# robertknight/rten

Measured on NVIDIA H100. Metric: resnet50_fp32_inferences_per_sec, higher is better.
Workload: dtype f32(tf32 mma, explicit opt-in)

## Files before the change

rten_b200/csrc/umma_gemm.cu:

```cuda
#include <cuda.h>
#include <cuda_runtime.h>

#include <algorithm>
#include <array>
#include <cmath>
#include <vector>
#include <cmath>
#include <cstdint>
#include <cstdio>
#include <cstdlib>

#include "math.cuh"
#include "ptx.cuh"
#include "rowops.h"
#include "umma_gemm.h"
#include "umma_kernel.cuh"

namespace rtb {

typedef CUresult (*EncodeTiledFn)(CUtensorMap*, CUtensorMapDataType, cuuint32_t, void*, const cuuint64_t*,
                                  const cuuint64_t*, const cuuint32_t*, const cuuint32_t*, CUtensorMapInterleave,
                                  CUtensorMapSwizzle, CUtensorMapL2promotion, CUtensorMapFloatOOBfill);

static EncodeTiledFn get_encode(rten_ctx* ctx) {
// ... 18 lines not shown
        }
    }
    for (int i = 0; i < rank; i++)
        if (od.dims[i] < 1 || od.dims[i] > 0xFFFFFFFFll) return false;
    return true;
}

bool encode_map(rten_ctx* ctx, CUtensorMap* map, const OperandDesc& od, int esize, bool is_f32,
                const uint32_t box[4], const uint32_t estr[4]) {
    EncodeTiledFn enc = get_encode(ctx);
    if (!enc) return false;
    cuuint64_t dims[4];
    cuuint64_t strides[3];
    cuuint32_t b[4], es[4];
    for (int i = 0; i < 4; i++) {
        dims[i] = (cuuint64_t)od.dims[i];
        b[i] = box[i];
        es[i] = estr[i];
    }
    for (int i = 1; i < 4; i++) {
        long long s = od.strides[i] * esize;
        if (s == 0 || od.dims[i] == 1) s = 16;
        strides[i - 1] = (cuuint64_t)s;
    }
    CUresult r = enc(map, is_f32 ? CU_TENSOR_MAP_DATA_TYPE_FLOAT32 : CU_TENSOR_MAP_DATA_TYPE_UINT8, 4,
                     const_cast<void*>(od.base), dims, strides, b, es, CU_TENSOR_MAP_INTERLEAVE_NONE,
                     CU_TENSOR_MAP_SWIZZLE_128B, CU_TENSOR_MAP_L2_PROMOTION_L2_256B,
                     CU_TENSOR_MAP_FLOAT_OOB_FILL_NONE);
    return r == CUDA_SUCCESS;
}

static void pick_conv_tile(const ConvGeom& g, int& tw, int& th, int& tb) {
    double best = -1.0;
    tw = th = tb = 1;
    for (int w = 1; w <= std::min(g.OW, 128); w++) {
        if (w * g.sx > 256) break;
        for (int h = 1; h <= std::min(g.OH, 128 / w); h++) {
            if (h * g.sy > 256) break;
            int b = std::min(g.B, 128 / (w * h));
            if (b < 1) continue;
            long long tiles = (long long)((g.OW + w - 1) / w) * ((g.OH + h - 1) / h) * ((g.B + b - 1) / b);
            double eff = (double)g.B * g.OH * g.OW / ((double)tiles * 128.0);
            if (eff > best + 1e-9 || (eff > best - 1e-9 && w > tw)) {
                best = eff;
                tw = w;
                th = h;
                tb = b;
            }
        }
    }
}

struct Plan {
    int bn = 32, splitk = 1, nbuf = 1;
    bool halo = false;
    int T = 0;
};

static Plan halo_plan(int bn, int T) {
    Plan pl;
    pl.halo = true;
    pl.bn = bn;
    pl.T = T;
    return pl;
}

struct Prepared {
    KParams p;
    uint32_t abox[4], aes[4], bbox_k;
    uint32_t pbox[4], pes[4];
    uint32_t a_rows;
    long long batch;
    OperandDesc od, ord;
    uint32_t dbox[4];
    int tma_store, res_tma;
    int wide;
    int chain_bytes;
    int step;
    int esize, kelems;
};

constexpr int SK_CNT_INTS = 1 << 16;
static int smem_budget_for(int n_stg) { return 227 * 1024 - SMEM_FIXED_BYTES - n_stg * STG_BYTES; }
static int wide_stages(int stage_bytes, int chain_bytes) {
    return std::min(MAX_STAGES, (227 * 1024 - WIDE_SMEM_FIXED_BYTES - chain_bytes) / stage_bytes);
}
static bool is_wide(int bn) { return bn > ACC_STRIDE; }

static Epi pick_epilogue(const GemmLaunch& L, int tma_store, int res_tma, int splitk) {
    const EpilogueDesc& e = L.epi;
    auto aligned = [](const void* ptr) { return (reinterpret_cast<uintptr_t>(ptr) & 15) == 0; };
    bool fast = tma_store && (L.N % 32) == 0 && !getenv("RTEN_B200_NO_FAST") && e.bias_kind != 2 &&
                (e.r == nullptr || res_tma) && (e.bias_kind != 1 || aligned(e.bias));
    if (L.kind == 1)
        fast = fast && (!(e.za || e.za8) || aligned(e.colsum)) && (!e.zb || e.zb_len == 1 || (e.zb_len == L.N && aligned(e.zb))) &&
               (!e.scale || e.scale_len == 1 || (e.scale_len == L.N && aligned(e.scale)));
    if (!fast) return Epi::Generic;
    const bool gelu = e.act > 1;
    if (!getenv("RTEN_B200_NO_PLAIN") && e.act <= 7) {
        if (L.kind == 0 && e.alpha == 1.0f && !e.range && (e.r == nullptr || e.r_scale == 1.0f))
            return gelu ? Epi::PlainF32Gelu : Epi::PlainF32;
        if (L.kind == 1 && e.scale && !e.za && !e.zb && (e.scale_len == 1 || e.scale_len == L.N) && splitk == 1 &&
            (!e.za8 || e.colsum))
            return gelu ? Epi::PlainI8Gelu : Epi::PlainI8;
    }
    return gelu ? Epi::FastGelu : Epi::Fast;
}

static const char* epi_name(Epi v) {
    static const char* const names[] = {"Generic", "Fast", "FastGelu", "PlainF32", "PlainF32Gelu", "PlainI8", "PlainI8Gelu"};
    return names[(int)v];
}

static bool is_plain_f32(Epi v) { return v == Epi::PlainF32 || v == Epi::PlainF32Gelu; }

struct PlanShape {
    long long tiles_n, units_m, tiles, units;
    int kb_per, stage_bytes, stages, n_stg;
};

static bool plan_shape(const Prepared& q, const Plan& pl, PlanShape& ps) {
    const KParams& p = q.p;
    if (pl.splitk < 1) return false;
    if (is_wide(pl.bn)) {
        if ((pl.bn != 128 && pl.bn != 256) || !q.wide || pl.splitk != 1) return false;
        if (pl.bn == 256 && q.p.epi.act > 1) return false;
    } else if (pl.bn < 16 || pl.bn % 32 || pl.bn % q.step) {
        return false;
    }
    if (pl.nbuf < (q.res_tma ? 2 : 1) || pl.nbuf > 4) return false;
    ps.tiles_n = q.chain_bytes ? 1 : (p.N + pl.bn - 1) / pl.bn;
    ps.units_m = p.tiles_m;
    ps.tiles = ps.units_m * ps.tiles_n * q.batch;
    ps.units = ps.tiles * pl.splitk;
    if (ps.units > 0x7FFFFFFFll) return false;
    ps.kb_per = (p.k_blocks + pl.splitk - 1) / pl.splitk;
    if (pl.splitk > 1) {
        if (pl.bn % 32 || (long long)(pl.splitk - 1) * ps.kb_per >= p.k_blocks) return false;
        if (ps.tiles * 2 > SK_CNT_INTS) return false;
    }
    ps.n_stg = 2 * pl.nbuf;
    ps.stage_bytes = A_STAGE_BYTES + pl.bn * KBYTES;
    ps.stages = is_wide(pl.bn) ? wide_stages(ps.stage_bytes, q.chain_bytes) : std::min(MAX_STAGES, smem_budget_for(ps.n_stg) / ps.stage_bytes);
    if (ps.stages < 2) return false;
    return true;
}

static double plan_cost(const Prepared& q, const Plan& pl, const PlanShape& ps, int num_sms) {
    const double active = (double)std::min<long long>(ps.units, num_sms);
    const double waves = std::ceil((double)ps.units / num_sms);
    const double bw = std::min(64.0, 7400.0 / active);
    const double mmas = 4.0;
    const double t_kb = std::max(mmas * std::max(42.0, (double)pl.bn), ps.stage_bytes / bw);
    double t_stage = std::max(t_kb, 320.0 + mmas * 42.0);
    t_stage = std::max(t_stage, 2300.0 / ps.stages);
    const double mainloop = ps.kb_per * t_stage;
    const double epi = is_wide(pl.bn) ? (pl.bn / 32.0) * 400.0 + 600.0 : (pl.bn / 32.0) * 350.0 / 2.0 + 600.0;
    double unit = (is_wide(pl.bn) ? mainloop + epi : std::max(mainloop, epi)) + 1500.0;
    double cost = waves * unit + 2500.0;
    if (pl.splitk > 1) cost += epi * (1.0 + 0.25 * pl.splitk) + 1500.0;

    return cost;
}

static void enumerate_plans(const Prepared& q, int num_sms, std::vector<std::pair<double, Plan>>& out) {
    const KParams& p = q.p;
    const int nmax = (p.N + q.step - 1) / q.step * q.step;
    static const int splits[] = {1, 2, 3, 4, 5, 6, 8, 10, 12, 16};
    for (int bn : {32, 64, 128, 256}) {
        if (bn > nmax && bn != 32) break;
        for (int sk : splits) {
            Plan pl;
            pl.bn = bn;
            pl.splitk = sk;
            if (sk > 1 && p.k_blocks / sk < 4) continue;
            const int kb_per = (p.k_blocks + sk - 1) / sk;
            pl.nbuf = (q.res_tma || kb_per < 24) ? 2 : 1;
            PlanShape ps;
            if (is_wide(bn)) {
                pl.nbuf = 2;
            } else if (pl.nbuf == 2) {
                PlanShape ps2;
                const bool ok2 = plan_shape(q, pl, ps2);
                pl.nbuf = 3;
                if (!plan_shape(q, pl, ps) || (ps.stages < 3 && !(ok2 && ps.stages == ps2.stages))) pl.nbuf = 2;
            }
            if (!plan_shape(q, pl, ps)) continue;
            if (sk > 1 && ps.tiles >= 2 * num_sms) continue;
            if (ps.stages < 2) continue;
            out.emplace_back(plan_cost(q, pl, ps, num_sms), pl);
        }
    }
    std::sort(out.begin(), out.end(), [](const std::pair<double, Plan>& x, const std::pair<double, Plan>& y) {
        return x.first < y.first;
    });
}

static rten_status prepare_launch(rten_ctx* ctx, const GemmLaunch& L, Prepared& q) {
    const int esize = L.kind == 0 ? 4 : 1;
    const int kelems = KBYTES / esize;
    if (!tma_compatible(L.a, esize, 4) || !tma_compatible(L.b, esize, 4)) return RTEN_ERR_UNSUPPORTED_VALUE;
    if (L.M <= 0 || L.N <= 0 || L.K <= 0) return RTEN_ERR_UNSUPPORTED_VALUE;
    q.esize = esize;
    q.kelems = kelems;
    KParams& p = q.p;
    memset(&p, 0, sizeof(p));
    p.M = L.M;
    p.N = L.N;
    p.K = L.K;
    p.z0 = L.z0;
    p.z1 = L.z1;
    p.kelems = kelems;
    p.conv = L.conv;
    p.epi = L.epi;
    p.c_blocks = 1;
    p.kw = 1;
    for (int i = 0; i < 4; i++) q.aes[i] = 1;
    if (L.conv) {
        const ConvGeom& g = L.g;
        pick_conv_tile(g, p.tw, p.th, p.tb);
        p.tiles_x = (g.OW + p.tw - 1) / p.tw;
        p.tiles_y = (g.OH + p.th - 1) / p.th;
        int tiles_b = (g.B + p.tb - 1) / p.tb;
        p.tiles_m = p.tiles_x * p.tiles_y * tiles_b;
        p.OH = g.OH;
        p.OW = g.OW;
        p.Bn = g.B;
        p.sy = g.sy;
        p.sx = g.sx;
        p.dy = g.dy;
        p.dx = g.dx;
        p.pt = g.pt;
        p.pl = g.pl;
        p.kw = g.kw;
        p.c_blocks = (g.C + kelems - 1) / kelems;
        p.k_blocks = g.kh * g.kw * p.c_blocks;
        p.z0 = p.z1 = 1;
        q.abox[0] = kelems;
        q.abox[1] = p.tw * g.sx;
        q.abox[2] = p.th * g.sy;
        q.abox[3] = p.tb;
        q.aes[1] = g.sx;
        q.aes[2] = g.sy;
        q.a_rows = p.tw * p.th * p.tb;
        q.batch = 1;
    } else {
        p.tiles_m = (L.M + BM - 1) / BM;
        p.k_blocks = (L.K + kelems - 1) / kelems;
        q.abox[0] = kelems;
        q.abox[1] = BM;
        q.abox[2] = 1;
        q.abox[3] = 1;
        q.a_rows = BM;
        q.batch = (long long)L.z0 * L.z1;
        p.a_bcast0 = (L.a.dims[2] == 1 && L.z0 > 1) ? 1 : 0;
        p.a_bcast1 = (L.a.dims[3] == 1 && L.z1 > 1) ? 1 : 0;
        p.b_bcast0 = (L.b.dims[2] == 1 && L.z0 > 1) ? 1 : 0;
        p.b_bcast1 = (L.b.dims[3] == 1 && L.z1 > 1) ? 1 : 0;
    }
    OperandDesc& od = q.od;
    OperandDesc& ord = q.ord;
    q.dbox[0] = 32;
    q.dbox[1] = q.dbox[2] = q.dbox[3] = 1;
// ... 85 lines not shown
    }
    return RTEN_OK;
}

static rten_status launch_plan(rten_ctx* ctx, const GemmLaunch& L, const Prepared& q, const Plan& pl, bool verbose,
                               void* ws = nullptr) {
    PlanShape ps;
    if (!plan_shape(q, pl, ps)) return RTEN_ERR_UNSUPPORTED_VALUE;
    KParams p = q.p;
    p.bn = pl.bn;
    p.splitk = pl.splitk;
    p.nbuf = pl.nbuf;
    p.tma_store = q.tma_store;
    p.res_tma = q.res_tma ? 1 : 0;
    p.kb_per = ps.kb_per;
    p.tiles_n = (int)ps.tiles_n;
    p.tiles_total = (int)ps.tiles;
    p.units_total = (int)ps.units;
    p.d_tiles_n.set(p.tiles_n);
    p.d_tiles_m.set(p.tiles_m);
    p.d_z0.set(p.z0);
    p.d_tiles_x.set(p.conv ? p.tiles_x : 1);
    p.d_tiles_y.set(p.conv ? p.tiles_y : 1);
    p.d_tiles_total.set(p.tiles_total);
    p.d_c_blocks.set(p.c_blocks);
    p.d_kw.set(p.kw);
    p.d_tw.set(p.conv ? p.tw : 1);
    p.d_th.set(p.conv ? p.th : 1);
    p.stage_bytes = ps.stage_bytes;
    p.tx_bytes = q.a_rows * KBYTES + p.bn * KBYTES;
    p.stages = ps.stages;
    p.sgn = L.kind == 0 ? 0 : (L.a_signed ? 1 : 0) | (L.b_signed ? 2 : 0);
    if (p.splitk > 1) {
        RTB_TRY(ensure_splitk_counters(ctx));
        if (!ws) RTB_TRY(temp_alloc(ctx, splitk_ws_bytes(ps, pl), &ws));
        p.sk_ws = reinterpret_cast<uint32_t*>(ws);
        p.sk_cnt = reinterpret_cast<int*>(ctx->sk_counters);
    }

    uint32_t bbox[4] = {(uint32_t)q.kelems, (uint32_t)p.bn, 1, 1}, bes[4] = {1, 1, 1, 1}, des[4] = {1, 1, 1, 1};
    TmaMaps m;
    if (!encode_map(ctx, &m.a, L.a, q.esize, L.kind == 0, q.abox, q.aes)) return RTEN_ERR_UNSUPPORTED_VALUE;
    if (!encode_map(ctx, &m.b, L.b, q.esize, L.kind == 0, bbox, bes)) return RTEN_ERR_UNSUPPORTED_VALUE;
    m.d = m.r = m.a2 = m.a_proj = m.b_proj = m.a2_proj = m.w2 = m.z = m.a;
    p.x3_cb = L.x3_cb;
    if (L.x3_cb && !encode_map(ctx, &m.a2, L.a_lo, q.esize, true, q.abox, q.aes)) return RTEN_ERR_UNSUPPORTED_VALUE;
    if (p.kb_proj) {
        p.x3_cb_proj = L.proj.x3_cb;
        if (!encode_map(ctx, &m.a_proj, L.proj.a, 4, true, q.pbox, q.pes) ||
            !encode_map(ctx, &m.b_proj, L.proj.b, 4, true, bbox, bes) ||
            (L.proj.x3_cb && !encode_map(ctx, &m.a2_proj, L.proj.a_lo, 4, true, q.pbox, q.pes)))
            return RTEN_ERR_UNSUPPORTED_VALUE;
    }
    if (p.tma_store && !encode_map(ctx, &m.d, q.od, 4, true, q.dbox, des)) {
        p.tma_store = 0;
        p.res_tma = 0;
        m.d = m.a;
    }
    if (p.res_tma && !encode_map(ctx, &m.r, q.ord, 4, true, q.dbox, des)) {
        p.res_tma = 0;
        m.r = m.a;
    }
    const Epi epi = pick_epilogue(L, p.tma_store, p.res_tma, p.splitk);
    if (epi == Epi::Generic && (L.kind == 1 || L.epi.act > 1)) p.res_tma = 0;
    if (q.chain_bytes) {
        const GemmLaunch::Chain& c = L.chain;
        const uint32_t wbox[4] = {32, (uint32_t)c.N2, 1, 1}, zbox[4] = {32, q.dbox[1], q.dbox[2], q.dbox[3]};
        if (epi != Epi::PlainF32 || (L.epi.r && !p.res_tma) || !encode_map(ctx, &m.w2, c.w, 4, true, wbox, des) ||
            !encode_map(ctx, &m.z, c.z, 4, true, zbox, des))
            return RTEN_ERR_UNSUPPORTED_VALUE;
        p.chain_n2 = c.N2;
        p.chain_passes = (L.N + p.bn - 1) / p.bn;
        p.chain_act = c.act;
        p.chain_bias = c.bias;
    }

    if (verbose)
        fprintf(stderr, "[umma_gemm] kind=%d conv=%d M=%d N=%d K=%d kb=%d kb_proj=%d tiles_m=%d bn=%d splitk=%d units=%d stages=%d tma_store=%d res_tma=%d nbuf=%d box=%dx%dx%d epi=%s%s\n",
                L.kind, L.conv, L.M, L.N, L.K, p.k_blocks, p.kb_proj, p.tiles_m, p.bn, p.splitk, p.units_total, p.stages,
                p.tma_store, p.res_tma, p.nbuf, p.tw, p.th, p.tb, epi_name(epi),
                p.chain_n2 == 64 ? " chain=64" : p.chain_n2 == 128 ? " chain=128" : "");
    if ((is_wide(p.bn) || p.kb_proj || L.epi.bias2) && !is_plain_f32(epi)) return RTEN_ERR_UNSUPPORTED_VALUE;
    const size_t smem_bytes = (size_t)p.stages * p.stage_bytes + q.chain_bytes +
                              (is_wide(p.bn) ? WIDE_SMEM_FIXED_BYTES : ps.n_stg * STG_BYTES + SMEM_FIXED_BYTES);
    using Kernel = void (*)(TmaMaps, KParams);
    static const Kernel narrow[2][7] = {
        {umma_gemm_kernel<0, Epi::Generic>, umma_gemm_kernel<0, Epi::Fast>, umma_gemm_kernel<0, Epi::FastGelu>,
         umma_gemm_kernel<0, Epi::PlainF32>, umma_gemm_kernel<0, Epi::PlainF32Gelu>, nullptr, nullptr},
        {umma_gemm_kernel<1, Epi::Generic>, umma_gemm_kernel<1, Epi::Fast>, umma_gemm_kernel<1, Epi::FastGelu>, nullptr,
         nullptr, umma_gemm_kernel<1, Epi::PlainI8>, umma_gemm_kernel<1, Epi::PlainI8Gelu>}};
    const Kernel kern = !is_wide(p.bn)              ? narrow[L.kind][(int)epi]
                        : p.chain_n2 == 64         ? umma_wide_kernel<Epi::PlainF32, 64>
                        : p.chain_n2 == 128        ? umma_wide_kernel<Epi::PlainF32, 128>
                        : epi == Epi::PlainF32Gelu ? umma_wide_kernel<Epi::PlainF32Gelu>
                                                   : umma_wide_kernel<Epi::PlainF32>;

    const int threads = is_wide(p.bn) ? WIDE_THREADS : NUM_THREADS;
    return launch(ctx, "umma_gemm launch", kern, {std::min(p.units_total, ctx->num_sms), threads, smem_bytes, 227 * 1024, true}, m, p);
}

static std::vector<long long> tune_key(const GemmLaunch& L, const Prepared& q) {
    const EpilogueDesc& e = L.epi;
    std::vector<long long> k = {L.kind, L.conv, L.M, L.N, L.K, L.z0, L.z1, q.tma_store, q.res_tma, e.act, e.bias_kind,
                                e.r != nullptr, (e.za != nullptr || e.za8 != nullptr), e.zb != nullptr, e.scale != nullptr,
                                L.a.strides[1], L.b.strides[1], L.x3_cb};
    if (L.conv) {
        const ConvGeom& g = L.g;
        for (long long v : {g.B, g.H, g.W, g.C, g.OH, g.OW, g.kh, g.kw, g.sy, g.sx, g.dy, g.dx, g.pt, g.pl}) k.push_back(v);
    }
    if (L.proj.C > 0) {
        const GemmLaunch::Projection& pr = L.proj;
        for (int64_t v : {(int64_t)-1, (int64_t)pr.C, (int64_t)pr.stride, (int64_t)pr.x3_cb, pr.a.dims[1], pr.a.dims[2],
                          pr.a.strides[1], pr.a.strides[2], pr.a.strides[3], pr.b.strides[1]})
            k.push_back(v);
    }
    return k;
}

static std::array<int, 3> plan_record(const Plan& pl) {
    return pl.halo ? std::array<int, 3>{-1, pl.bn, pl.T} : std::array<int, 3>{pl.bn, pl.splitk, pl.nbuf};
}

static Plan plan_from_record(const std::array<int, 3>& r) {
    if (r[0] < 0) return halo_plan(r[1], r[2]);
    Plan pl;
    pl.bn = r[0];
    pl.splitk = r[1];
    pl.nbuf = r[2];
    return pl;
}

void tune_cache_load(rten_ctx* ctx, const char* path) {
    FILE* f = fopen(path, "r");
    if (!f) return;
    char line[2048];
    while (fgets(line, sizeof(line), f)) {
        std::vector<long long> key;
        std::array<int, 3> plan{};
        char* p = line;
        bool in_plan = false;
        int np = 0;
        while (*p) {
            while (*p == ' ') p++;
            if (*p == '|') {
                in_plan = true;
                p++;
                continue;
            }
            if (*p == '\n' || *p == 0) break;
            char* end = nullptr;
            const long long v = strtoll(p, &end, 10);
            if (end == p) break;
            if (in_plan) {
                if (np < 3) plan[np] = (int)v;
                np++;
            } else {
                key.push_back(v);
            }
            p = end;
        }
        if (np == 3 && !key.empty()) ctx->tune_cache[key] = plan;
    }
    fclose(f);
}

void tune_cache_save(rten_ctx* ctx, const char* path) {
    FILE* f = fopen(path, "w");
// ... 111 lines not shown
    for (size_t i = 0; i < ncand; i++) {
        PlanShape ps;
        if (plan_shape(q, cands[i].second, ps)) ws_max = std::max(ws_max, splitk_ws_bytes(ps, cands[i].second));
    }
    void* ws = nullptr;
    if (ws_max) {
        RTB_TRY(ensure_splitk_counters(ctx));
        RTB_TRY(temp_alloc(ctx, ws_max, &ws));
        cudaStreamSynchronize(ctx->stream);
    }
    cudaEvent_t e0, e1;
    cudaEventCreate(&e0);
    cudaEventCreate(&e1);
    auto time_plan = [&](const Plan& x, int n) -> double {
        if (run_plan(ctx, L, q, x, false, ws) != RTEN_OK) return -1.0;
        cudaEventRecord(e0, ctx->stream);
        bool ok = true;
        for (int r = 0; r < n && ok; r++) ok = run_plan(ctx, L, q, x, false, ws) == RTEN_OK;
        cudaEventRecord(e1, ctx->stream);
        if (cudaEventSynchronize(e1) != cudaSuccess || !ok) return -1.0;
        float t = 0.f;
        cudaEventElapsedTime(&t, e0, e1);
        return (double)t / n;
    };
    double best_ms = 1e30;
    int reps = 4;
    std::vector<std::pair<double, size_t>> timed;
    for (size_t i = 0; i < ncand; i++) {
        const Plan& x = cands[i].second;
        double ms = time_plan(x, reps);
        if (ms < 0) continue;
        timed.emplace_back(ms, i);
        if (verbose)
            fprintf(stderr, "[autotune] bn=%d splitk=%d nbuf=%d model=%.0f -> %.2f us\n", x.bn, x.splitk, x.nbuf,
                    cands[i].first, ms * 1e3);
        if (ms < best_ms) {
            best_ms = ms;
            plan = x;
        }
        reps = std::max(4, std::min(32, (int)(0.15 / std::max(best_ms, 1e-3))));
    }
    std::sort(timed.begin(), timed.end());
    best_ms = 1e30;
    for (size_t k = 0; k < std::min<size_t>(3, timed.size()); k++) {
        const Plan& x = cands[timed[k].second].second;
        const double again = time_plan(x, 2 * reps);
        const double ms = again < 0 ? timed[k].first : again;
        if (ms < best_ms) {
            best_ms = ms;
            plan = x;
        }
    }
    for (const auto& s : HALO_SHAPES) {
        const Plan x = halo_plan(s[0], s[1]);
        if (!halo || x.bn > L.N) continue;
        double ms = time_plan(x, reps);
        if (ms > 0 && ms < best_ms * 1.05) ms = time_plan(x, 2 * reps);
        if (verbose && ms > 0) fprintf(stderr, "[autotune] halo bn=%d T=%d -> %.2f us\n", x.bn, x.T, ms * 1e3);
        if (ms > 0 && ms < best_ms * 0.97) {
            best_ms = ms;
            plan = x;
        }
    }
    cudaEventDestroy(e0);
    cudaEventDestroy(e1);
    ctx->tune_cache[tune_key(L, q)] = plan_record(plan);
    return RTEN_OK;
}

rten_status launch_umma_gemm(rten_ctx* ctx, const GemmLaunch& L) {
    const bool verbose = getenv("RTEN_B200_VERBOSE") != nullptr;
    const char* force_bn = getenv("RTEN_B200_FORCE_BN");
    const char* force_sk = getenv("RTEN_B200_FORCE_SPLITK");
    const char* halo_on = getenv("RTEN_B200_HALO");
    const bool halo = L.conv && L.kind == 0 && L.g.kh * L.g.kw > 1 && !L.x3_cb && !L.proj.C && !getenv("RTEN_B200_NO_HALO");
    Prepared q;
    if (L.chain.N2 > 0) {
        if (L.kind != 0 || ctx->f32_mode != RTEN_F32_TF32 || L.x3_cb || getenv("RTEN_B200_NO_CHAIN"))
            return RTEN_ERR_UNSUPPORTED_VALUE;
        RTB_TRY(prepare_launch(ctx, L, q));
        Plan pl;
        pl.bn = 128;
        pl.nbuf = 2;
        return launch_plan(ctx, L, q, pl, verbose);
    }
    if (L.kind == 0 && ctx->f32_mode == RTEN_F32_TF32X3) return launch_tf32x3(ctx, L);
    int hbn, hT;
    if (halo && halo_on && atoi(halo_on) != 0 && halo_model_shape(ctx, L, hbn, hT)) {
        const rten_status hs = run_plan(ctx, L, q, halo_plan(hbn, hT), verbose);
        if (hs != RTEN_ERR_UNSUPPORTED_VALUE) return hs;
    }
    RTB_TRY(prepare_launch(ctx, L, q));
    const bool forced = force_bn || force_sk;
    if (!forced && !ctx->tune_cache.empty()) {
        auto hit = ctx->tune_cache.find(tune_key(L, q));
        if (hit != ctx->tune_cache.end()) {
            const Plan pl = plan_from_record(hit->second);
            PlanShape ps;
            if (pl.halo ? halo && halo_shape_fits(L, pl.bn, pl.T) : plan_shape(q, pl, ps)) return run_plan(ctx, L, q, pl, verbose);
            if (verbose) fprintf(stderr, "[umma_gemm] recorded plan no longer valid for this problem: re-planning\n");
            ctx->tune_cache.erase(hit);
        }
    }
    std::vector<std::pair<double, Plan>> cands;
    enumerate_plans(q, ctx->num_sms, cands);
    if (cands.empty()) return RTEN_ERR_UNSUPPORTED_VALUE;
    Plan plan = cands[0].second;
    if (forced) {
        bool found = false;
        for (const auto& c : cands) {
            const Plan& x = c.second;
            if (force_bn && x.bn != atoi(force_bn)) continue;
            if (force_sk && x.splitk != atoi(force_sk)) continue;
            plan = x;
            found = true;
            break;
        }
        if (!found) {
            ctx->forced_misses++;
            if (verbose) fprintf(stderr, "[umma_gemm] no valid plan matches the forced fields: using the model's choice\n");
            if (getenv("RTEN_B200_FORCE_STRICT"))
                return fail(ctx, RTEN_ERR_INVALID_VALUE, "no launch plan matches the forced RTEN_B200_FORCE_* fields");
        } else {
            ctx->forced_hits++;
        }
    } else if (ctx->autotune) {
        RTB_TRY(autotune(ctx, L, q, cands, halo, verbose, plan));
    }
    return run_plan(ctx, L, q, plan, verbose);
}

}
```

rten_b200/csrc/umma_kernel.cuh:

```cuda
#pragma once
#include <cuda.h>
#include <cuda_runtime.h>

#include <cstdint>

#include "math.cuh"
#include "ptx.cuh"
#include "umma_gemm.h"

namespace rtb {

constexpr int BM = 128;
constexpr int KBYTES = 128;
constexpr int A_STAGE_BYTES = BM * KBYTES;
constexpr int ACC_STRIDE = 64;
constexpr int PRODUCER_WARP = 12;
constexpr int NUM_THREADS = 416;
constexpr int STG_BYTES = 128 * 128;
constexpr int MAX_STAGES = 8;

struct FastDiv {
    uint32_t d = 1, mul = 0, shr = 0;
    __host__ void set(int div) {
        d = (uint32_t)(div < 1 ? 1 : div);
// ... 95 lines not shown
    switch (n) {
        case 0: asm volatile("cp.async.bulk.wait_group.read 0;" ::: "memory"); break;
        case 1: asm volatile("cp.async.bulk.wait_group.read 1;" ::: "memory"); break;
        case 2: asm volatile("cp.async.bulk.wait_group.read 2;" ::: "memory"); break;
        default: asm volatile("cp.async.bulk.wait_group.read 3;" ::: "memory"); break;
    }
}

__device__ __forceinline__ int f32_to_ordered(float f) {
    const int i = __float_as_int(f);
    return i >= 0 ? i : i ^ 0x7fffffff;
}
__device__ __forceinline__ void range_commit(int* range, float lo, float hi) {
#pragma unroll
    for (int o = 16; o > 0; o >>= 1) {
        lo = fminf(lo, __shfl_xor_sync(0xffffffffu, lo, o));
        hi = fmaxf(hi, __shfl_xor_sync(0xffffffffu, hi, o));
    }
    if ((threadIdx.x & 31) == 0 && lo <= hi) {
        atomicMin(&range[0], f32_to_ordered(lo));
        atomicMax(&range[1], f32_to_ordered(hi));
    }
}

__device__ __noinline__ float4 act4(float4 x, int act, float alpha, float beta) {
    if (act == 2) {
        gelu_ref_x2(x.x, x.y);
        gelu_ref_x2(x.z, x.w);
        return x;
    }
    x.x = apply_act(x.x, act, alpha, beta);
    x.y = apply_act(x.y, act, alpha, beta);
    x.z = apply_act(x.z, act, alpha, beta);
    x.w = apply_act(x.w, act, alpha, beta);
    return x;
}

__device__ __forceinline__ bool splitk_publish(const KParams& p, int t, int ks, int grp, int q, int lane, uint32_t t_acc,
                                               int* flag, uint32_t acc_smem) {
    const int r = q * 32 + lane;
    const int nchunks = p.bn >> 5;
    for (int c0 = grp * 32; c0 < p.bn; c0 += 64) {
        uint32_t v[32];
        acc_ld(acc_smem, t_acc + c0, v);
        uint32_t* w = p.sk_ws + ((((size_t)t * p.splitk + ks) * nchunks + (c0 >> 5)) << 12) + r;
#pragma unroll
        for (int j = 0; j < 32; j++) __stcg(w + j * 128, v[j]);
    }
    __threadfence();
    asm volatile("bar.sync %0, 128;" ::"r"(1 + grp) : "memory");
    if (q == 0 && lane == 0) {
        int* cnt = p.sk_cnt + t * 2 + grp;
        const int old = atomicAdd(cnt, 1);
        const int last = old == p.splitk - 1;
        if (last) *cnt = 0;
        __threadfence();
        *flag = last;
    }
    asm volatile("bar.sync %0, 128;" ::"r"(1 + grp) : "memory");
    return *reinterpret_cast<volatile int*>(flag) != 0;
}

template <int KIND>
__device__ __forceinline__ void splitk_sum(const KParams& p, int t, int c0, int r, uint32_t (&v)[32]) {
    const int nchunks = p.bn >> 5;
    const uint32_t* w = p.sk_ws + ((((size_t)t * p.splitk) * nchunks + (c0 >> 5)) << 12) + r;
    const size_t stride = (size_t)nchunks << 12;
#pragma unroll
    for (int j = 0; j < 32; j++) v[j] = __ldcg(w + j * 128);
#pragma unroll 1
    for (int s = 1; s < p.splitk; s++) {
        w += stride;
#pragma unroll
        for (int j = 0; j < 32; j++) {
            const uint32_t x = __ldcg(w + j * 128);
            if (KIND == 0)
                v[j] = __float_as_uint(__fadd_rn(__uint_as_float(v[j]), __uint_as_float(x)));
            else
                v[j] += x;
        }
    }
}

struct SmemLayout {
    uint8_t* smem;
    uint64_t *full_bar, *empty_bar, *acc_full, *acc_empty, *res_bar, *w_bar;
    int* sk_flag;
    float* bias;
    uint32_t acc_smem;
};

}

#include "umma_epilogue.cuh"

namespace rtb {

template <int KIND, int SGN, int N>
__device__ __forceinline__ void mma_units(const KParams& p, const SmemLayout& L, int worker, int n_workers) {
    const int lane = threadIdx.x & 31;
    const uint32_t smem0 = smem_u32(L.smem);
    uint32_t ring = 0, aphase = 0;
    int stage = 0;
    for (int u = worker, it = 0; u < p.units_total; u += n_workers, it++) {
        const int kb0 = p.d_tiles_total.div(u) * p.kb_per, kb1 = min(p.k_blocks, kb0 + p.kb_per);
        const int acc = it & 1;
        acc_t<KIND> d0[N / 2], d1[N / 2];
#pragma unroll
        for (int i = 0; i < N / 2; i++) d0[i] = d1[i] = 0;
        int prev = -1;
        for (int kb = kb0; kb < kb1; kb++) {
            mbar_wait(&L.full_bar[stage], (ring >> stage) & 1);
            wgmma_fence_operand(d0);
            wgmma_fence_operand(d1);
            wgmma_fence();
            const uint32_t sa = smem0 + stage * p.stage_bytes;
            const uint64_t adesc = make_kmajor_sw128_desc(sa);
            const uint64_t bdesc = make_kmajor_sw128_desc(sa + A_STAGE_BYTES);
#pragma unroll
            for (int k = 0; k < 4; k++) {
                wgmma_k<KIND, SGN, N>(d0, adesc + 2 * k, bdesc + 2 * k);
                wgmma_k<KIND, SGN, N>(d1, adesc + (64 * KBYTES >> 4) + 2 * k, bdesc + 2 * k);
            }
            wgmma_commit();
            wgmma_fence_operand(d0);
            wgmma_fence_operand(d1);
            wgmma_wait<1>();
            if (prev >= 0 && lane == 0) mbar_arrive(&L.empty_bar[prev]);
            prev = stage;
            ring ^= 1u << stage;
            if (++stage == p.stages) stage = 0;
        }
        wgmma_wait<0>();
        wgmma_fence_operand(d0);
        wgmma_fence_operand(d1);
        if (prev >= 0 && lane == 0) mbar_arrive(&L.empty_bar[prev]);
        mbar_wait(&L.acc_empty[acc], ((aphase >> acc) & 1) ^ 1);
        aphase ^= 1u << acc;
        acc_store_frag<N>(L.acc_smem, d0, 0, acc * ACC_STRIDE);
        acc_store_frag<N>(L.acc_smem, d1, 64, acc * ACC_STRIDE);
        mbar_arrive(&L.acc_full[acc]);
    }
}

template <int KIND, int N>
__device__ __forceinline__ void mma_role(const KParams& p, const SmemLayout& L, int worker, int n_workers) {
    if (KIND == 0) mma_units<KIND, 0, N>(p, L, worker, n_workers);
    else if (p.sgn == 0) mma_units<KIND, 0, N>(p, L, worker, n_workers);
    else if (p.sgn == 1) mma_units<KIND, 1, N>(p, L, worker, n_workers);
    else if (p.sgn == 2) mma_units<KIND, 2, N>(p, L, worker, n_workers);
    else mma_units<KIND, 3, N>(p, L, worker, n_workers);
}

struct TmaMaps {
    CUtensorMap a, b, d, r, a2, a_proj, b_proj, a2_proj, w2, z;
};

__device__ __forceinline__ void prefetch_maps(const TmaMaps& m, const KParams& p) {
    tma_prefetch_desc(&m.a);
    tma_prefetch_desc(&m.b);
    if (p.tma_store) tma_prefetch_desc(&m.d);
    if (p.res_tma) tma_prefetch_desc(&m.r);
    if (p.x3_cb) tma_prefetch_desc(&m.a2);
    if (p.kb_proj) {
        tma_prefetch_desc(&m.a_proj);
        tma_prefetch_desc(&m.b_proj);
        if (p.x3_cb_proj) tma_prefetch_desc(&m.a2_proj);
    }
}

template <bool CHAIN = false>
__device__ __forceinline__ void producer_role(const KParams& p, const TmaMaps& m, const SmemLayout& L, int worker,
// ... 71 lines not shown
                cb = 0;
                tap++;
                if (++kx == p.kw) {
                    kx = 0;
                    ky++;
                }
            }
            __syncwarp();
            ring ^= 1u << stage;
            if (++stage == p.stages) stage = 0;
        }
      }
    }
}

constexpr int SMEM_FIXED_BYTES = 1024  + 4096  + ACC_SMEM_BYTES;
static_assert(ACC_SMEM_BYTES % 1024 == 0, "operand stages must stay 1024-B aligned");
static_assert(2 * ACC_STRIDE <= ACC_COLS, "two accumulator stages");

__device__ __forceinline__ SmemLayout carve_smem(uint8_t* smem_raw) {
    uint8_t* base = reinterpret_cast<uint8_t*>((reinterpret_cast<uintptr_t>(smem_raw) + 1023) & ~uintptr_t(1023));
    SmemLayout L;
    L.full_bar = reinterpret_cast<uint64_t*>(base);
    L.empty_bar = L.full_bar + MAX_STAGES;
    L.acc_full = L.empty_bar + MAX_STAGES;
    L.acc_empty = L.acc_full + 2;
    L.res_bar = L.acc_empty + 2;
    L.sk_flag = reinterpret_cast<int*>(L.res_bar + 8) + 2;
    L.bias = reinterpret_cast<float*>(base + 1024);
    L.acc_smem = smem_u32(base + 4096);
    L.smem = base + 4096 + ACC_SMEM_BYTES;
    return L;
}

__device__ __forceinline__ void kernel_setup(const SmemLayout& L) {
    const int warp = threadIdx.x >> 5;
    const int lane = threadIdx.x & 31;
    if (warp == PRODUCER_WARP) {
        if (lane < MAX_STAGES) {
            mbar_init(&L.full_bar[lane], 1);
            mbar_init(&L.empty_bar[lane], 4);
        }
        fence_mbar_init();
        __syncwarp();
        asm volatile("bar.arrive 15, %0;" ::"r"(NUM_THREADS) : "memory");
        return;
    }
    if (warp == 1) {
        if (lane < 2)
            mbar_init(&L.acc_full[lane], 128);
        else if (lane < 4)
            mbar_init(&L.acc_empty[lane - 2], 8);
        else if (lane < 12)
            mbar_init(&L.res_bar[lane - 4], 1);
        fence_mbar_init();
    }
    asm volatile("bar.sync 15, %0;" ::"r"(NUM_THREADS) : "memory");
}

template <int KIND, Epi E>
__global__ void __launch_bounds__(NUM_THREADS, 1)
umma_gemm_kernel(const __grid_constant__ TmaMaps m, const __grid_constant__ KParams p) {
    extern __shared__ uint8_t smem_raw[];
    const SmemLayout L = carve_smem(smem_raw);
    if (threadIdx.x == 0) prefetch_maps(m, p);
    kernel_setup(L);
    if (threadIdx.x >> 5 != PRODUCER_WARP) pdl_wait();
    pdl_launch_dependents();
    const int worker = (int)blockIdx.x, n_workers = (int)gridDim.x;
    const int warp = threadIdx.x >> 5;
    if (warp == PRODUCER_WARP) {
        producer_role(p, m, L, worker, n_workers);
    } else if (warp < 4) {
        if (p.bn == 32)
            mma_role<KIND, 32>(p, L, worker, n_workers);
        else
            mma_role<KIND, 64>(p, L, worker, n_workers);
    } else {
        epilogue<KIND, E>(p, L, &m.d, &m.r, worker, n_workers);
    }
}

constexpr int WIDE_THREADS = 384;
constexpr int WIDE_SMEM_FIXED_BYTES = 1024 + 2 * STG_BYTES + 2048;

template <int N>
__device__ __forceinline__ void wgmma_wide(float (&d)[N / 2], uint64_t adesc, uint64_t bdesc) {
    if constexpr (N == 128) wgmma_tf32_n128(d, adesc, bdesc);
    else wgmma_tf32_n256(d, adesc, bdesc);
}

__device__ __forceinline__ void consumers_sync() { asm volatile("bar.sync 1, 256;" ::: "memory"); }

__device__ __forceinline__ int chain_w_bytes(const KParams& p) { return (p.N / 32) * p.chain_n2 * KBYTES; }

template <bool CHAIN>
__device__ __forceinline__ SmemLayout carve_wide_smem(uint8_t* smem_raw, const KParams& p) {
    uint8_t* base = reinterpret_cast<uint8_t*>((reinterpret_cast<uintptr_t>(smem_raw) + 1023) & ~uintptr_t(1023));
    uint8_t* tail = base + (size_t)p.stages * p.stage_bytes + (CHAIN ? chain_w_bytes(p) : 0) + 2 * STG_BYTES;
    SmemLayout L;
    L.smem = base;
    L.full_bar = reinterpret_cast<uint64_t*>(tail);
    L.empty_bar = L.full_bar + MAX_STAGES;
    L.res_bar = L.empty_bar + MAX_STAGES;
    L.w_bar = L.res_bar + 2;
    L.acc_full = L.acc_empty = nullptr;
    L.sk_flag = nullptr;
    L.bias = reinterpret_cast<float*>(tail + 256);
    L.acc_smem = 0;
    return L;
}

template <int N>
__device__ __forceinline__ void wide_main_loop(const KParams& p, const SmemLayout& L, float (&d)[N / 2], int wg, int lane,
                                               int& stage, uint32_t& ring) {
    const uint32_t smem0 = smem_u32(L.smem);
#pragma unroll
    for (int i = 0; i < N / 2; i++) d[i] = 0.0f;
    int prev = -1;
    for (int kb = 0; kb < p.k_blocks; kb++) {
        mbar_wait(&L.full_bar[stage], (ring >> stage) & 1);
        wgmma_fence_operand(d);
        wgmma_fence();
        const uint32_t sa = smem0 + stage * p.stage_bytes;
        const uint64_t adesc = make_kmajor_sw128_desc(sa + wg * (64 * KBYTES));
        const uint64_t bdesc = make_kmajor_sw128_desc(sa + A_STAGE_BYTES);
#pragma unroll
        for (int k = 0; k < 4; k++) wgmma_wide<N>(d, adesc + 2 * k, bdesc + 2 * k);
        wgmma_commit();
        wgmma_fence_operand(d);
        wgmma_wait<1>();
        if (prev >= 0 && lane == 0) mbar_arrive(&L.empty_bar[prev]);
        prev = stage;
        ring ^= 1u << stage;
        if (++stage == p.stages) stage = 0;
    }
    wgmma_wait<0>();
    wgmma_fence_operand(d);
    if (prev >= 0 && lane == 0) mbar_arrive(&L.empty_bar[prev]);
}

template <Epi E, int NA>
__device__ __forceinline__ void stage_chunk(float (&d)[NA], int k, uint8_t* stg, const float* bias, bool valid, bool res,
                                            int act, int row0, int sw, int cq, float alpha = 0.0f, float beta = 0.0f) {
#pragma unroll
    for (int j = 0; j < 4; j++) {
        const int i0 = 16 * k + 4 * j;
        float2* px[2];
#pragma unroll
        for (int h = 0; h < 2; h++)
            px[h] = reinterpret_cast<float2*>(stg + (row0 + 8 * h) * 128 + (((2 * j + (cq >> 1)) ^ sw) << 4) + 8 * (cq & 1));
        if (valid) {
            const float2 bb = *reinterpret_cast<const float2*>(bias + 8 * j + 2 * cq);
#pragma unroll
            for (int h = 0; h < 2; h++) {
                uint32_t v0 = __float_as_uint(d[i0 + 2 * h]), v1 = __float_as_uint(d[i0 + 2 * h + 1]);
                float2 rr = make_float2(0.f, 0.f);
                if (res) rr = *px[h];
                plain_f32_pair(v0, v1, res, rr, bb, act == 1);
                d[i0 + 2 * h] = __uint_as_float(v0);
                d[i0 + 2 * h + 1] = __uint_as_float(v1);
            }
            if (E == Epi::PlainF32Gelu) {
                const float4 g = act4(make_float4(d[i0], d[i0 + 1], d[i0 + 2], d[i0 + 3]), act, alpha, beta);
                d[i0] = g.x;
                d[i0 + 1] = g.y;
                d[i0 + 2] = g.z;
                d[i0 + 3] = g.w;
            }
        }
#pragma unroll
        for (int h = 0; h < 2; h++) *px[h] = make_float2(d[i0 + 2 * h], d[i0 + 2 * h + 1]);
    }
}

template <Epi E, int N>
__device__ __forceinline__ void wide_consumer(const KParams& p, const SmemLayout& L, const CUtensorMap* tma_d,
                                              const CUtensorMap* tma_r, int worker, int n_workers) {
    const int t = threadIdx.x - 128;
    const int wg = t >> 7;
    const int lane = threadIdx.x & 31;
    const int row0 = 64 * wg + 16 * ((t & 127) >> 5) + (lane >> 2);
    const int sw = lane >> 2;
    const int cq = lane & 3;
    const bool issuer = t == 0;
    const EpilogueDesc& e = p.epi;
    uint8_t* const stg0 = L.smem + (size_t)p.stages * p.stage_bytes;
    float* const bias_s = L.bias;
    uint32_t ring = 0, rphase = 0;
    uint32_t ci = 0;
    int stage = 0;
    auto load_residual = [&](const TileCoord& tc, int c0, int buf) {
        uint64_t* rb = &L.res_bar[buf];
        mbar_expect_tx(rb, p.res_tx_bytes);
        const int4 x = out_coord(p, tc, c0);
        tma_load_4d(stg0 + buf * STG_BYTES, tma_r, rb, x.x, x.y, x.z, x.w);
    };
    for (int u = worker; u < p.units_total; u += n_workers) {
        {
            const TileCoord tc = decode_tile(p, u);
            if (t < N) bias_s[t] = (e.bias_kind == 1 && tc.n0 + t < p.N) ? column_bias(e, tc.n0 + t) : 0.0f;
            if (issuer) {
                bulk_wait_read(0);
                if (p.res_tma) load_residual(tc, 0, ci & 1);
            }
        }
        float d[N / 2];
        wide_main_loop<N>(p, L, d, wg, lane, stage, ring);
        const TileCoord tc = decode_tile(p, u);
        consumers_sync();
#pragma unroll
        for (int k = 0; k < N / 32; k++, ci++) {
            const int buf = ci & 1;
            uint8_t* stg = stg0 + buf * STG_BYTES;
            const int nbase = tc.n0 + 32 * k;
            if (issuer) {
                bulk_wait_read(0);
                if (p.res_tma && k + 1 < N / 32) load_residual(tc, 32 * (k + 1), buf ^ 1);
            }
            if (p.res_tma) {
                mbar_wait(&L.res_bar[buf], (rphase >> buf) & 1);
                rphase ^= 1u << buf;
            }
            stage_chunk<E>(d, k, stg, bias_s + 32 * k, nbase < p.N, p.res_tma, e.act, row0, sw, cq, e.act_alpha, e.act_beta);
            fence_proxy_async();
            consumers_sync();
            if (issuer) {
                const int4 x = out_coord(p, tc, 32 * k);
                tma_store_4d(tma_d, stg, x.x, x.y, x.z, x.w);
                asm volatile("cp.async.bulk.commit_group;" ::: "memory");
            }
        }
    }
    if (issuer) asm volatile("cp.async.bulk.wait_group.read 0;" ::: "memory");
}

template <int N2>
__device__ __forceinline__ void wide_chain_consumer(const KParams& p, const SmemLayout& L, const TmaMaps& m, int worker,
                                                    int n_workers) {
    constexpr int N = 128;
    const int t = threadIdx.x - 128;
    const int wg = t >> 7;
    const int lane = threadIdx.x & 31;
    const int row0 = 64 * wg + 16 * ((t & 127) >> 5) + (lane >> 2);
    const int sw = lane >> 2;
    const int cq = lane & 3;
    const bool issuer = t == 0;
    const EpilogueDesc& e = p.epi;
    const uint32_t w2 = smem_u32(L.smem) + p.stages * p.stage_bytes;
    uint8_t* const stg0 = L.smem + (size_t)p.stages * p.stage_bytes + chain_w_bytes(p);
    float* const bias_s = L.bias;
    uint32_t ring = 0, rphase = 0;
    uint32_t ci = 0;
    int stage = 0;
    auto load_residual = [&](const TileCoord& tc, int c0, int buf) {
        uint64_t* rb = &L.res_bar[buf];
        mbar_expect_tx(rb, p.res_tx_bytes);
        const int4 x = out_coord(p, tc, c0);
        tma_load_4d(stg0 + buf * STG_BYTES, &m.r, rb, x.x, x.y, x.z, x.w);
    };
    auto chunk_barrier = [&](float (&acc2)[N2 / 2]) {
        wgmma_wait<0>();
        wgmma_fence_operand(acc2);
        if (issuer) bulk_wait_read(0);
        fence_proxy_async();
        consumers_sync();
    };
    mbar_wait(L.w_bar, 0);
    for (int u = worker; u < p.units_total; u += n_workers) {
        {
            const TileCoord tc = decode_tile(p, u);
            if (t < p.N) bias_s[t] = e.bias_kind == 1 ? column_bias(e, t) : 0.0f;
            if (t < N2) bias_s[256 + t] = p.chain_bias ? __ldg(p.chain_bias + t) : 0.0f;
            if (issuer && p.res_tma) load_residual(tc, 0, ci & 1);
        }
        float acc2[N2 / 2];
#pragma unroll
        for (int i = 0; i < N2 / 2; i++) acc2[i] = 0.0f;
        for (int pass = 0; pass < p.chain_passes; pass++) {
            float d[N / 2];
            wide_main_loop<N>(p, L, d, wg, lane, stage, ring);
            const TileCoord tc = decode_tile(p, u);
            consumers_sync();
#pragma unroll
            for (int k = 0; k < N / 32; k++) {
                const int c0 = N * pass + 32 * k;
                if (c0 >= p.N) break;
                const int buf = ci & 1;
                uint8_t* stg = stg0 + buf * STG_BYTES;
                if (p.res_tma) {
                    mbar_wait(&L.res_bar[buf], (rphase >> buf) & 1);
                    rphase ^= 1u << buf;
                }
                stage_chunk<Epi::PlainF32>(d, k, stg, bias_s + c0, true, p.res_tma, e.act, row0, sw, cq);
                chunk_barrier(acc2);
                if (issuer) {
                    const int4 x = out_coord(p, tc, c0);
                    tma_store_4d(&m.d, stg, x.x, x.y, x.z, x.w);
                    asm volatile("cp.async.bulk.commit_group;" ::: "memory");
                    if (p.res_tma && c0 + 32 < p.N) load_residual(tc, c0 + 32, buf ^ 1);
                }
                wgmma_fence();
                const uint64_t adesc = make_kmajor_sw128_desc(smem_u32(stg) + wg * (64 * KBYTES));
                const uint64_t bdesc = make_kmajor_sw128_desc(w2 + (c0 / 32) * (N2 * KBYTES));
#pragma unroll
                for (int kk = 0; kk < 4; kk++) {
                    if constexpr (N2 == 64) wgmma_tf32_n64(acc2, adesc + 2 * kk, bdesc + 2 * kk);
                    else wgmma_tf32_n128(acc2, adesc + 2 * kk, bdesc + 2 * kk);
                }
                wgmma_commit();
                wgmma_fence_operand(acc2);
                ci++;
            }
        }
        wgmma_wait<0>();
        wgmma_fence_operand(acc2);
        const TileCoord tc = decode_tile(p, u);
#pragma unroll
        for (int k = 0; k < N2 / 32; k++, ci++) {
            uint8_t* stg = stg0 + (ci & 1) * STG_BYTES;
            stage_chunk<Epi::PlainF32>(acc2, k, stg, bias_s + 256 + 32 * k, true, false, p.chain_act, row0, sw, cq);
            chunk_barrier(acc2);
            if (issuer) {
                tma_store_4d(&m.z, stg, 32 * k, tc.ox0, tc.oy0, tc.b0);
                asm volatile("cp.async.bulk.commit_group;" ::: "memory");
            }
        }
    }
    if (issuer) asm volatile("cp.async.bulk.wait_group.read 0;" ::: "memory");
}

template <Epi E, int CHAIN_N2 = 0>
__global__ void __launch_bounds__(WIDE_THREADS, 1)
umma_wide_kernel(const __grid_constant__ TmaMaps m, const __grid_constant__ KParams p) {
    extern __shared__ uint8_t smem_raw[];
    const SmemLayout L = carve_wide_smem<(CHAIN_N2 > 0)>(smem_raw, p);
    const int warp = threadIdx.x >> 5;
    const int lane = threadIdx.x & 31;
    if (threadIdx.x == 0) {
        prefetch_maps(m, p);
        if constexpr (CHAIN_N2 > 0) {
            tma_prefetch_desc(&m.w2);
            tma_prefetch_desc(&m.z);
        }
    }
    if (warp == 1) {
        if (lane < MAX_STAGES) {
            mbar_init(&L.full_bar[lane], 1);
            mbar_init(&L.empty_bar[lane], 8);
        } else if (lane < MAX_STAGES + (CHAIN_N2 > 0 ? 3 : 2)) {
            mbar_init(&L.res_bar[lane - MAX_STAGES], 1);
        }
        fence_mbar_init();
    }
    __syncthreads();
    if (warp >= 4) pdl_wait();
    pdl_launch_dependents();
    if (warp < 4) {
        asm volatile("setmaxnreg.dec.sync.aligned.u32 56;");
        if (warp == 0) producer_role<(CHAIN_N2 > 0)>(p, m, L, (int)blockIdx.x, (int)gridDim.x);
    } else {
        asm volatile("setmaxnreg.inc.sync.aligned.u32 224;");
        if constexpr (CHAIN_N2 > 0) {
            wide_chain_consumer<CHAIN_N2>(p, L, m, (int)blockIdx.x, (int)gridDim.x);
        } else {
            if (E == Epi::PlainF32Gelu || p.bn == 128)
                wide_consumer<E, 128>(p, L, &m.d, &m.r, (int)blockIdx.x, (int)gridDim.x);
            else
                wide_consumer<E, 256>(p, L, &m.d, &m.r, (int)blockIdx.x, (int)gridDim.x);
        }
    }
}

}
```

Baseline: 17320.

## Make wide-kernel epilogue staging buffer count variable and prefetch residuals via ring

Makes the number of epilogue staging buffers in the wide (bn 128/256) kernel a plan parameter (2-4) instead of a fixed two. Shared memory accounting and the planner are updated, so conv GEMMs without residual can pick deeper staging, and chained GEMMs with residual pick the deepest option that keeps 3 mainloop stages. In the chain consumer, residual TMA loads are issued several chunks ahead through a small shared-memory ring state machine that can cross unit boundaries. TMA store waits are relaxed to allow nbuf-2 outstanding stores. The aim is to overlap epilogue stores and residual loads with compute, at the cost of shared memory taken from mainloop stages.

Measured after the change: 17720 (median of 6 runs). +2.3%, better.

```diff
diff --git a/rten_b200/csrc/umma_gemm.cu b/rten_b200/csrc/umma_gemm.cu
--- a/rten_b200/csrc/umma_gemm.cu
+++ b/rten_b200/csrc/umma_gemm.cu
@@ -124,8 +124,8 @@
 
 constexpr int SK_CNT_INTS = 1 << 16;
 static int smem_budget_for(int n_stg) { return 227 * 1024 - SMEM_FIXED_BYTES - n_stg * STG_BYTES; }
-static int wide_stages(int stage_bytes, int chain_bytes) {
-    return std::min(MAX_STAGES, (227 * 1024 - WIDE_SMEM_FIXED_BYTES - chain_bytes) / stage_bytes);
+static int wide_stages(int stage_bytes, int chain_bytes, int nbuf) {
+    return std::min(MAX_STAGES, (227 * 1024 - WIDE_SMEM_FIXED_BYTES - nbuf * STG_BYTES - chain_bytes) / stage_bytes);
 }
 static bool is_wide(int bn) { return bn > ACC_STRIDE; }
 
@@ -170,7 +170,8 @@
     } else if (pl.bn < 16 || pl.bn % 32 || pl.bn % q.step) {
         return false;
     }
-    if (pl.nbuf < (q.res_tma ? 2 : 1) || pl.nbuf > 4) return false;
+    if (pl.nbuf < (q.res_tma || is_wide(pl.bn) ? 2 : 1) || pl.nbuf > 4) return false;
+    if (is_wide(pl.bn) && q.res_tma && !q.chain_bytes && pl.nbuf != 2) return false;
     ps.tiles_n = q.chain_bytes ? 1 : (p.N + pl.bn - 1) / pl.bn;
     ps.units_m = p.tiles_m;
     ps.tiles = ps.units_m * ps.tiles_n * q.batch;
@@ -183,7 +184,7 @@
     }
     ps.n_stg = 2 * pl.nbuf;
     ps.stage_bytes = A_STAGE_BYTES + pl.bn * KBYTES;
-    ps.stages = is_wide(pl.bn) ? wide_stages(ps.stage_bytes, q.chain_bytes) : std::min(MAX_STAGES, smem_budget_for(ps.n_stg) / ps.stage_bytes);
+    ps.stages = is_wide(pl.bn) ? wide_stages(ps.stage_bytes, q.chain_bytes, pl.nbuf) : std::min(MAX_STAGES, smem_budget_for(ps.n_stg) / ps.stage_bytes);
     if (ps.stages < 2) return false;
     return true;
 }
@@ -197,7 +198,8 @@
     double t_stage = std::max(t_kb, 320.0 + mmas * 42.0);
     t_stage = std::max(t_stage, 2300.0 / ps.stages);
     const double mainloop = ps.kb_per * t_stage;
-    const double epi = is_wide(pl.bn) ? (pl.bn / 32.0) * 400.0 + 600.0 : (pl.bn / 32.0) * 350.0 / 2.0 + 600.0;
+    const double epi = is_wide(pl.bn) ? (pl.bn / 32.0) * (pl.nbuf > 2 ? 300.0 : 400.0) + 600.0
+                                      : (pl.bn / 32.0) * 350.0 / 2.0 + 600.0;
     double unit = (is_wide(pl.bn) ? mainloop + epi : std::max(mainloop, epi)) + 1500.0;
     double cost = waves * unit + 2500.0;
     if (pl.splitk > 1) cost += epi * (1.0 + 0.25 * pl.splitk) + 1500.0;
@@ -220,7 +222,11 @@
             pl.nbuf = (q.res_tma || kb_per < 24) ? 2 : 1;
             PlanShape ps;
             if (is_wide(bn)) {
-                pl.nbuf = 2;
+                for (int nb = 2; nb <= (p.conv && !q.res_tma ? 4 : 2); nb++) {
+                    pl.nbuf = nb;
+                    if (plan_shape(q, pl, ps) && (nb == 2 || ps.stages >= 3)) out.emplace_back(plan_cost(q, pl, ps, num_sms), pl);
+                }
+                continue;
             } else if (pl.nbuf == 2) {
                 PlanShape ps2;
                 const bool ok2 = plan_shape(q, pl, ps2);
@@ -472,7 +478,7 @@
                 p.chain_n2 == 64 ? " chain=64" : p.chain_n2 == 128 ? " chain=128" : "");
     if ((is_wide(p.bn) || p.kb_proj || L.epi.bias2) && !is_plain_f32(epi)) return RTEN_ERR_UNSUPPORTED_VALUE;
     const size_t smem_bytes = (size_t)p.stages * p.stage_bytes + q.chain_bytes +
-                              (is_wide(p.bn) ? WIDE_SMEM_FIXED_BYTES : ps.n_stg * STG_BYTES + SMEM_FIXED_BYTES);
+                              (is_wide(p.bn) ? WIDE_SMEM_FIXED_BYTES + pl.nbuf * STG_BYTES : ps.n_stg * STG_BYTES + SMEM_FIXED_BYTES);
     using Kernel = void (*)(TmaMaps, KParams);
     static const Kernel narrow[2][7] = {
         {umma_gemm_kernel<0, Epi::Generic>, umma_gemm_kernel<0, Epi::Fast>, umma_gemm_kernel<0, Epi::FastGelu>,
@@ -750,6 +756,15 @@
         Plan pl;
         pl.bn = 128;
         pl.nbuf = 2;
+        for (int nb = 4; q.res_tma && nb > 2; nb--) {
+            Plan x = pl;
+            x.nbuf = nb;
+            PlanShape ps;
+            if (plan_shape(q, x, ps) && ps.stages >= 3) {
+                pl = x;
+                break;
+            }
+        }
         return launch_plan(ctx, L, q, pl, verbose);
     }
     if (L.kind == 0 && ctx->f32_mode == RTEN_F32_TF32X3) return launch_tf32x3(ctx, L);
diff --git a/rten_b200/csrc/umma_kernel.cuh b/rten_b200/csrc/umma_kernel.cuh
--- a/rten_b200/csrc/umma_kernel.cuh
+++ b/rten_b200/csrc/umma_kernel.cuh
@@ -201,12 +201,15 @@
     }
 }
 
+struct WideRing;
+
 struct SmemLayout {
     uint8_t* smem;
     uint64_t *full_bar, *empty_bar, *acc_full, *acc_empty, *res_bar, *w_bar;
     int* sk_flag;
     float* bias;
     uint32_t acc_smem;
+    WideRing* ring;
 };
 
 }
@@ -444,7 +447,7 @@
 }
 
 constexpr int WIDE_THREADS = 384;
-constexpr int WIDE_SMEM_FIXED_BYTES = 1024 + 2 * STG_BYTES + 2048;
+constexpr int WIDE_SMEM_FIXED_BYTES = 1024 + 2048;
 
 template <int N>
 __device__ __forceinline__ void wgmma_wide(float (&d)[N / 2], uint64_t adesc, uint64_t bdesc) {
@@ -459,13 +462,14 @@
 template <bool CHAIN>
 __device__ __forceinline__ SmemLayout carve_wide_smem(uint8_t* smem_raw, const KParams& p) {
     uint8_t* base = reinterpret_cast<uint8_t*>((reinterpret_cast<uintptr_t>(smem_raw) + 1023) & ~uintptr_t(1023));
-    uint8_t* tail = base + (size_t)p.stages * p.stage_bytes + (CHAIN ? chain_w_bytes(p) : 0) + 2 * STG_BYTES;
+    uint8_t* tail = base + (size_t)p.stages * p.stage_bytes + (CHAIN ? chain_w_bytes(p) : 0) + (size_t)p.nbuf * STG_BYTES;
     SmemLayout L;
     L.smem = base;
     L.full_bar = reinterpret_cast<uint64_t*>(tail);
     L.empty_bar = L.full_bar + MAX_STAGES;
     L.res_bar = L.empty_bar + MAX_STAGES;
-    L.w_bar = L.res_bar + 2;
+    L.w_bar = L.res_bar + 4;
+    L.ring = reinterpret_cast<WideRing*>(L.w_bar + 1);
     L.acc_full = L.acc_empty = nullptr;
     L.sk_flag = nullptr;
     L.bias = reinterpret_cast<float*>(tail + 256);
@@ -534,6 +538,43 @@
 #pragma unroll
         for (int h = 0; h < 2; h++) *px[h] = make_float2(d[i0 + 2 * h], d[i0 + 2 * h + 1]);
     }
+}
+
+struct WideRing {
+    int unit, k, buf;
+    uint32_t next;
+    uint32_t stored;
+};
+
+__device__ __forceinline__ void ring_start(WideRing* r, int worker) {
+    r->unit = worker;
+    r->k = r->buf = 0;
+    r->next = r->stored = 0;
+}
+
+__device__ __noinline__ void ring_request(WideRing* r, const KParams& p, const CUtensorMap* tma_r, uint8_t* stg0,
+                                          uint64_t* res_bar, int ahead, int per_unit, int with_res, int n_workers) {
+    int unit = r->unit, k = r->k, buf = r->buf;
+    uint32_t next = r->next;
+    const uint32_t stored = r->stored, end = stored + ahead;
+    for (; next < end && unit < p.units_total; next++) {
+        if (k < with_res) {
+            if (next >= (uint32_t)p.nbuf) bulk_wait_read((int)(stored + p.nbuf - 1 - next));
+            uint64_t* rb = &res_bar[buf];
+            mbar_expect_tx(rb, p.res_tx_bytes);
+            const int4 x = out_coord(p, decode_tile(p, unit), 32 * k);
+            tma_load_4d(stg0 + buf * STG_BYTES, tma_r, rb, x.x, x.y, x.z, x.w);
+        }
+        if (++buf == p.nbuf) buf = 0;
+        if (++k == per_unit) {
+            k = 0;
+            unit += n_workers;
+        }
+    }
+    r->unit = unit;
+    r->k = k;
+    r->buf = buf;
+    r->next = next;
 }
 
 template <Epi E, int N>
@@ -550,41 +591,42 @@
     uint8_t* const stg0 = L.smem + (size_t)p.stages * p.stage_bytes;
     float* const bias_s = L.bias;
     uint32_t ring = 0, rphase = 0;
-    uint32_t ci = 0;
+    int buf = 0;
     int stage = 0;
-    auto load_residual = [&](const TileCoord& tc, int c0, int buf) {
-        uint64_t* rb = &L.res_bar[buf];
+    auto load_residual = [&](const TileCoord& tc, int c0, int b) {
+        uint64_t* rb = &L.res_bar[b];
         mbar_expect_tx(rb, p.res_tx_bytes);
         const int4 x = out_coord(p, tc, c0);
-        tma_load_4d(stg0 + buf * STG_BYTES, tma_r, rb, x.x, x.y, x.z, x.w);
+        tma_load_4d(stg0 + b * STG_BYTES, tma_r, rb, x.x, x.y, x.z, x.w);
     };
     for (int u = worker; u < p.units_total; u += n_workers) {
         {
             const TileCoord tc = decode_tile(p, u);
             if (t < N) bias_s[t] = (e.bias_kind == 1 && tc.n0 + t < p.N) ? column_bias(e, tc.n0 + t) : 0.0f;
-            if (issuer) {
+            if (issuer && p.res_tma) {
                 bulk_wait_read(0);
-                if (p.res_tma) load_residual(tc, 0, ci & 1);
+                load_residual(tc, 0, buf);
             }
         }
         float d[N / 2];
         wide_main_loop<N>(p, L, d, wg, lane, stage, ring);
         const TileCoord tc = decode_tile(p, u);
+        if (issuer && !p.res_tma) bulk_wait_read(p.nbuf - 1);
         consumers_sync();
 #pragma unroll
-        for (int k = 0; k < N / 32; k++, ci++) {
-            const int buf = ci & 1;
+        for (int k = 0; k < N / 32; k++) {
             uint8_t* stg = stg0 + buf * STG_BYTES;
             const int nbase = tc.n0 + 32 * k;
-            if (issuer) {
-                bulk_wait_read(0);
-                if (p.res_tma && k + 1 < N / 32) load_residual(tc, 32 * (k + 1), buf ^ 1);
-            }
             if (p.res_tma) {
+                if (issuer) {
+                    bulk_wait_read(0);
+                    if (k + 1 < N / 32) load_residual(tc, 32 * (k + 1), buf ^ 1);
+                }
                 mbar_wait(&L.res_bar[buf], (rphase >> buf) & 1);
                 rphase ^= 1u << buf;
             }
             stage_chunk<E>(d, k, stg, bias_s + 32 * k, nbase < p.N, p.res_tma, e.act, row0, sw, cq, e.act_alpha, e.act_beta);
+            if (issuer && !p.res_tma) bulk_wait_read(p.nbuf - 2);
             fence_proxy_async();
             consumers_sync();
             if (issuer) {
@@ -592,6 +634,7 @@
                 tma_store_4d(tma_d, stg, x.x, x.y, x.z, x.w);
                 asm volatile("cp.async.bulk.commit_group;" ::: "memory");
             }
+            if (++buf == p.nbuf) buf = 0;
         }
     }
     if (issuer) asm volatile("cp.async.bulk.wait_group.read 0;" ::: "memory");
@@ -609,33 +652,36 @@
     const int cq = lane & 3;
     const bool issuer = t == 0;
     const EpilogueDesc& e = p.epi;
+    const int nbuf = p.nbuf;
+    const int y_chunks = p.N / 32, unit_chunks = y_chunks + N2 / 32;
     const uint32_t w2 = smem_u32(L.smem) + p.stages * p.stage_bytes;
     uint8_t* const stg0 = L.smem + (size_t)p.stages * p.stage_bytes + chain_w_bytes(p);
     float* const bias_s = L.bias;
     uint32_t ring = 0, rphase = 0;
-    uint32_t ci = 0;
+    int buf = 0;
     int stage = 0;
-    auto load_residual = [&](const TileCoord& tc, int c0, int buf) {
-        uint64_t* rb = &L.res_bar[buf];
-        mbar_expect_tx(rb, p.res_tx_bytes);
-        const int4 x = out_coord(p, tc, c0);
-        tma_load_4d(stg0 + buf * STG_BYTES, &m.r, rb, x.x, x.y, x.z, x.w);
-    };
     auto chunk_barrier = [&](float (&acc2)[N2 / 2]) {
         wgmma_wait<0>();
         wgmma_fence_operand(acc2);
-        if (issuer) bulk_wait_read(0);
+        if (issuer) bulk_wait_read(nbuf - 2);
         fence_proxy_async();
         consumers_sync();
     };
+    auto next_chunk = [&]() {
+        if (++buf == nbuf) buf = 0;
+        if (issuer) {
+            L.ring->stored++;
+            if (p.res_tma) ring_request(L.ring, p, &m.r, stg0, L.res_bar, nbuf - 1, unit_chunks, y_chunks, n_workers);
+        }
+    };
     mbar_wait(L.w_bar, 0);
+    if (issuer) {
+        ring_start(L.ring, worker);
+        if (p.res_tma) ring_request(L.ring, p, &m.r, stg0, L.res_bar, nbuf - 1, unit_chunks, y_chunks, n_workers);
+    }
     for (int u = worker; u < p.units_total; u += n_workers) {
-        {
-            const TileCoord tc = decode_tile(p, u);
-            if (t < p.N) bias_s[t] = e.bias_kind == 1 ? column_bias(e, t) : 0.0f;
-            if (t < N2) bias_s[256 + t] = p.chain_bias ? __ldg(p.chain_bias + t) : 0.0f;
-            if (issuer && p.res_tma) load_residual(tc, 0, ci & 1);
-        }
+        if (t < p.N) bias_s[t] = e.bias_kind == 1 ? column_bias(e, t) : 0.0f;
+        if (t < N2) bias_s[256 + t] = p.chain_bias ? __ldg(p.chain_bias + t) : 0.0f;
         float acc2[N2 / 2];
 #pragma unroll
         for (int i = 0; i < N2 / 2; i++) acc2[i] = 0.0f;
@@ -648,7 +694,6 @@
             for (int k = 0; k < N / 32; k++) {
                 const int c0 = N * pass + 32 * k;
                 if (c0 >= p.N) break;
-                const int buf = ci & 1;
                 uint8_t* stg = stg0 + buf * STG_BYTES;
                 if (p.res_tma) {
                     mbar_wait(&L.res_bar[buf], (rphase >> buf) & 1);
@@ -660,8 +705,8 @@
                     const int4 x = out_coord(p, tc, c0);
                     tma_store_4d(&m.d, stg, x.x, x.y, x.z, x.w);
                     asm volatile("cp.async.bulk.commit_group;" ::: "memory");
-                    if (p.res_tma && c0 + 32 < p.N) load_residual(tc, c0 + 32, buf ^ 1);
                 }
+                next_chunk();
                 wgmma_fence();
                 const uint64_t adesc = make_kmajor_sw128_desc(smem_u32(stg) + wg * (64 * KBYTES));
                 const uint64_t bdesc = make_kmajor_sw128_desc(w2 + (c0 / 32) * (N2 * KBYTES));
@@ -672,21 +717,21 @@
                 }
                 wgmma_commit();
                 wgmma_fence_operand(acc2);
-                ci++;
             }
         }
         wgmma_wait<0>();
         wgmma_fence_operand(acc2);
         const TileCoord tc = decode_tile(p, u);
 #pragma unroll
-        for (int k = 0; k < N2 / 32; k++, ci++) {
-            uint8_t* stg = stg0 + (ci & 1) * STG_BYTES;
+        for (int k = 0; k < N2 / 32; k++) {
+            uint8_t* stg = stg0 + buf * STG_BYTES;
             stage_chunk<Epi::PlainF32>(acc2, k, stg, bias_s + 256 + 32 * k, true, false, p.chain_act, row0, sw, cq);
             chunk_barrier(acc2);
             if (issuer) {
                 tma_store_4d(&m.z, stg, 32 * k, tc.ox0, tc.oy0, tc.b0);
                 asm volatile("cp.async.bulk.commit_group;" ::: "memory");
             }
+            next_chunk();
         }
     }
     if (issuer) asm volatile("cp.async.bulk.wait_group.read 0;" ::: "memory");
@@ -710,7 +755,7 @@
         if (lane < MAX_STAGES) {
             mbar_init(&L.full_bar[lane], 1);
             mbar_init(&L.empty_bar[lane], 8);
-        } else if (lane < MAX_STAGES + (CHAIN_N2 > 0 ? 3 : 2)) {
+        } else if (lane < MAX_STAGES + (CHAIN_N2 > 0 ? 5 : 4)) {
             mbar_init(&L.res_bar[lane - MAX_STAGES], 1);
         }
         fence_mbar_init();
```
